# fulcrumgenomics/fgumi

Measured on AMD Instinct MI355X. Metric: simplex consensus throughput, input raw reads/s (depth-8 x 150bp), higher is better.
Workload: dtype f64

## Files before the change

fgumi_amd/csrc/api.cpp:

```cpp
#include <chrono>
#include <cstdio>
#include <stdexcept>
#include <cstring>
#include <mutex>
#include <map>
#include <mutex>
#include <string>
#include <thread>
#include "engine.h"
#include <gnu/libc-version.h>
#include <cmath>
#include "fastpath.h"
#include "host_common.h"
#include "simgen.h"
#include "canon_core.h"
#include "reject_core.h"
#include "aln_tags_core.h"

namespace fgx {
uint32_t launch_canon_molecules(hipStream_t s, bool codec, const canon::Params& P, const canon::CodecParams& PC, const uint8_t* d_blob,
                                const uint64_t* d_rec_off, const uint32_t* d_rec_len, const uint32_t* d_grp_first, const uint32_t* d_def, uint32_t nd,
                                const uint64_t* d_first, uint8_t* d_out, const uint64_t* d_out_off, uint32_t* d_out_len, int* d_status,
                                canon::Delta* d_delta, DevBuf& slabs);
void canon_layout_device(hipStream_t s, const uint32_t* d_rec_len, const uint32_t* d_grp_first, const uint32_t* d_def, uint32_t nd, unsigned long long* work,
// ... 1272 lines not shown
  double run = 0.0;
  for (uint32_t i = 0; i < n; i++) { run += (double)weights[i]; acc[i] = run; }
  const double total = acc[n - 1];
  for (uint32_t k = 1; k < world; k++) {
    const double want = total * (double)k / (double)world;
    const uint32_t idx = (uint32_t)(std::lower_bound(acc.begin(), acc.end(), want) - acc.begin());
    uint32_t c = idx + 1 > n ? n : idx + 1;
    if (c < cuts[k - 1]) c = cuts[k - 1];
    cuts[k] = c;
  }
  cuts[world] = n;
  for (uint32_t k = 1; k <= world; k++) if (cuts[k] < cuts[k - 1]) cuts[k] = cuts[k - 1];
  return 0;
}
uint32_t fgx_debug_last_split_chunks(const fgx_caller* c) { return (c && c->fast) ? c->fast->fp.last_split_chunks : 0u; }
uint32_t fgx_debug_last_big_families(const fgx_caller* c) { return (c && c->fast) ? c->fast->fp.last_big_families : 0u; }
uint32_t fgx_debug_last_meth_device(const fgx_caller* c) { return (c && c->fast) ? c->fast->fp.last_meth_device : 0u; }
uint32_t fgx_debug_last_deep_families(const fgx_caller* c) { return (c && c->fast) ? c->fast->fp.last_deep_families : 0u; }
void fgx_debug_last_split_builds(const fgx_caller* c, uint64_t* out4) {
  if (!out4) return;
  out4[0] = out4[1] = out4[2] = out4[3] = 0;
  if (c && c->fast) { const FastPath& f = c->fast->fp; out4[0] = f.last_packed_families; out4[1] = f.last_classic_families; out4[2] = f.last_split_build; out4[3] = f.last_first_stage_retries; }
}
void fgx_debug_last_chain(const fgx_caller* c, uint32_t* out2) { if (out2) { out2[0] = (c && c->fast) ? c->fast->fp.last_launches : 0u; out2[1] = (c && c->fast) ? c->fast->fp.last_host_syncs : 0u; } }
uint32_t fgx_debug_last_routed(const fgx_caller* c) { return (c && c->fast) ? c->fast->fp.last_routed : 0u; }
int fgx_debug_last_direct(const fgx_caller* c) { return (c && c->fast) ? c->fast->fp.last_direct : 0; }
void fgx_set_general_only(fgx_caller* c, int on) { if (c) c->general_only = on != 0; }
void fgx_set_fast_lds_bytes(fgx_caller* c, uint32_t bytes) { if (c) { if (!c->fast) c->fast = new FastState(); c->fast->fp.lds_tile_bytes_large = bytes; } }

int fgx_call_columns(fgx_caller* c, const uint8_t* bases, const uint8_t* quals, uint32_t n_cols, uint32_t depth, uint8_t* out_base,
                     uint8_t* out_qual, uint32_t* out_depth, uint32_t* out_errors) {
  if (!c) return 1;
  c->err.clear();
  try {
    ColumnBatch& B = c->batch;
    B.clear();
    std::vector<uint8_t> rb, rq;
    for (uint32_t j0 = 0; j0 < n_cols; j0 += 4096) {
      uint32_t w = std::min<uint32_t>(4096, n_cols - j0);
      uint32_t rd0 = (uint32_t)B.reads.size();
      for (uint32_t i = 0; i < depth; i++) {
        rb.resize(w); rq.resize(w);
        for (uint32_t k = 0; k < w; k++) { rb[k] = bases[(size_t)(j0 + k) * depth + i]; rq[k] = quals[(size_t)(j0 + k) * depth + i]; }
        B.add_read(rb.data(), rq.data(), w);
      }
      if (depth == 0) { B.add_job(rd0, 0, w); continue; }
// ... 129 lines not shown
```

fgumi_amd/csrc/fastpath.h:

```cpp
#pragma once
#include "engine.h"

namespace fgx {

constexpr int FAST_RX_CAP = 48;

struct EndDesc {
  uint64_t col_off;
  uint64_t first_off;
  uint64_t kept_off;
  uint32_t cons_len;
  uint32_t rec_size;
  uint16_t mi_off, cb_off;
  uint8_t mi_len, cb_len, rx_len, type;
  uint8_t has_cb, has_rx, valid, meth;
  char rx[FAST_RX_CAP];
};
struct MethSlot { uint32_t std_size, n_ml, mm_len, _pad; };

struct DuplexDesc {
  uint64_t a_off, b_off;
  uint32_t len;
  uint32_t first_rec;
  uint32_t cb_rec;
// ... 158 lines not shown
  uint32_t n_deferred; const uint32_t* d_deferred;
  const uint64_t* d_out_off;
  const uint64_t* d_slot_size;
  uint32_t n_slots;
  double ms_kernels, ms_k_family, ms_k_emit; uint64_t cols_used; uint64_t full_items;
};

struct FastPath {
  DevBuf d_ends, d_sizes, d_offsets, d_code, d_qual, d_depth, d_err, d_misc, d_deferred, d_out, d_scan_tmp, d_strings;
  uint32_t lds_tile_bytes = 12288;
  uint32_t lds_tile_bytes_large = 65536;
  DevBuf d_retry, d_bound, d_colbase, d_statslots, d_full_items, d_full_count, d_obs, d_obs_all, d_retry2, d_retry_old;
  DevBuf d_w2img;
  DevBuf d_famdesc;
  DevBuf d_fwimg;
  DevBuf d_split_rec, d_split_fam, d_split_out, d_route, d_s2img;
  DevBuf d_big;
  uint32_t last_big_families = 0;
  uint32_t last_deep_families = 0;
  DevBuf d_deep_sizes, d_deep_row0, d_deep_rows, d_deep_fams, d_deep_out, d_deep_out2;
  DevBuf d_mflag, d_mu, d_mt, d_mslot, d_mcontigs;
  uint32_t last_meth_device = 0;
  uint32_t last_routed = 0;
  uint64_t last_packed_families = 0, last_classic_families = 0;
  uint32_t last_split_build = 0;
  uint32_t last_first_stage_retries = 0;
  uint32_t last_launches = 0, last_host_syncs = 0;
  DevBuf d_dir_size, d_dir_off, d_dir_base, d_slot_desc, d_slot_err, d_out2, d_scan_tmp2;
  bool direct_off = false;
  uint64_t dir_cap_min = 0;
  uint32_t dir_chunks_run = 0;
  int last_direct = 0;
  uint32_t lds_wave_bytes = 6144;
  uint32_t lds_wave_bytes_duplex = 8704;
  uint32_t lds_wave_bytes_codec = 5120;
  hipEvent_t ev[4] = {nullptr, nullptr, nullptr, nullptr};
  uint32_t pool_slack = 256; bool pool_init = false;
  uint32_t pool_div = 8;
  static constexpr int RUN_AGAIN_LARGER_POOL = -77;
  bool lds_attr_set = false, s2_attr_set = false, v2_attr_set = false;
  static constexpr int MAX_CHUNKS = 65;
  uint32_t last_split_chunks = 0;
  hipStream_t s2 = nullptr;
  hipEvent_t ev_chunk[MAX_CHUNKS] = {}, ev_cols[MAX_CHUNKS] = {}, ev_fin = nullptr, ev_sample = nullptr;
  int run(fgx_caller* c, const uint8_t* d_blob, uint64_t blob_len, const uint64_t* d_rec_off, const uint32_t* d_rec_len, uint32_t n_rec,
          const uint32_t* d_grp_first, uint32_t n_grp, FastResult* res);
// ... 5 lines not shown
```

fgumi_amd/csrc/fastpath.hip:

```cpp
#if !defined(FGX_WAVEMU)
#include <hipcub/hipcub.hpp>
#endif
#include "bamrec.h"
#include "engine.h"
#include <cstdlib>
#include <memory>
#include <string>
#include <type_traits>
#include "fastpath.h"
#include "gate_core.h"
#include "packed_core.h"

#if defined(FGX_WAVEMU)
#define FGX_DYN_LDS(name) uint8_t* const name = wavemu::dyn_lds()
#define FGX_PIN(...) ((void)0)
#define FGX_UNDEF4(a, b, c, d) do { a = 0; b = 0; c = 0; d = 0; } while (0)
#define FGX_MEM_PIN() ((void)0)
#define FGX_CONST_AS
#else
#define FGX_DYN_LDS(name) extern __shared__ __align__(16) uint8_t name[]
#define FGX_PIN(...) asm volatile("" : __VA_ARGS__)
#define FGX_UNDEF4(a, b, c, d) asm volatile("" : "=v"(a), "=v"(b), "=v"(c), "=v"(d))
#define FGX_MEM_PIN() asm volatile("" ::: "memory")
#define FGX_CONST_AS __attribute__((address_space(4)))
#endif

namespace fgx {
// ... 3855 lines not shown
    hip_check(hipcub::DeviceScan::ExclusiveSum(fp.d_scan_tmp.p, tb, in, out, (int)n, s), what);
  }
  template <class Image> const void* table_image(DevBuf& d, void (*build)(Image&, const ConsensusTables&), const char* what) {
    if (!d.p) {
      const auto img = std::make_unique<Image>();
      build(*img, c->h_tables.t);
      d.reserve(sizeof(Image));
      hip_check(hipMemcpyAsync(d.p, img.get(), sizeof(Image), hipMemcpyHostToDevice, s), what);
      sync();
    }
    return d.p;
  }
  FastParams stage_params(uint32_t bytes, bool retry) {
    hip_check(hipMemsetAsync(cnt(MISC_N_RETRY), 0, 4, s), "memset");
    FastParams PS = P;
    PS.group_list = cur_list; PS.lds_wave_bytes = bytes;
    PS.retry = retry ? lists[out_list] : nullptr; PS.n_retry = cnt(MISC_N_RETRY);
    return PS;
  }
  void next_list(uint32_t n) { cur_list = lists[out_list]; n_cur = n; out_list ^= 1; }

  void set_up() {
    fp.last_meth_device = 0; fp.last_direct = 0; fp.last_split_chunks = 0;
    fp.last_routed = 0; fp.last_big_families = 0; fp.last_deep_families = 0; fp.last_packed_families = 0; fp.last_classic_families = 0; fp.last_split_build = 0; fp.last_first_stage_retries = 0;
    fp.d_ends.reserve((size_t)n_slots * (duplex ? sizeof(DuplexDesc) : codec ? sizeof(CodecDesc) : sizeof(EndDesc)));
    fp.d_sizes.reserve(((size_t)n_slots + 1) * 8);
    fp.d_offsets.reserve(((size_t)n_slots + 1) * 8);
    fp.d_deferred.reserve((size_t)n_grp * 4);
    fp.d_misc.reserve(MISC_WORDS * 8);
    hip_check(hipMemsetAsync(fp.d_misc.p, 0, MISC_WORDS * 8, s), "memset");
    misc = fp.d_misc.as<unsigned long long>();
    const std::string strs = c->prefix + c->rg;
    fp.d_strings.reserve(strs.size() + 16);
    if (!strs.empty()) hip_check(hipMemcpyAsync(fp.d_strings.p, strs.data(), strs.size(), hipMemcpyHostToDevice, s), "H2D strings");
    for (int i = 0; i < 4; i++) if (!fp.ev[i]) hip_check(hipEventCreate(&fp.ev[i]), "hipEventCreate");
    fp.d_bound.reserve(((size_t)n_grp + 1) * 8); fp.d_colbase.reserve(((size_t)n_grp + 1) * 8);
    fp.d_statslots.reserve((size_t)STAT_SLOTS * 32 * 8);
    hip_check(hipMemsetAsync(fp.d_statslots.p, 0, (size_t)STAT_SLOTS * 32 * 8, s), "memset");
    fp.d_famdesc.reserve((size_t)n_grp * 16);
    hip_check(hipEventRecord(c->ev0, s), "event");
    hip_check(hipEventRecord(fp.ev[0], s), "event");
    fpw = mean_recs >= 1.0 ? (uint32_t)(64.0 / mean_recs) : 16u;
    fpw = fpw < 1u ? 1u : fpw > 16u ? 16u : fpw;
    if (sw.split_fpw) fpw = sw.split_fpw;
    n_chunks = ps.chunks >= 1 ? (uint32_t)ps.chunks : std::min<uint32_t>(8u, std::max<uint32_t>(1u, n_grp / 150000u));
    if (n_chunks > (uint32_t)FastPath::MAX_CHUNKS - 1) n_chunks = FastPath::MAX_CHUNKS - 1;
    chunk_fam_raw = (n_grp + n_chunks - 1) / n_chunks;
// ... 515 lines not shown
    };
    read_counters();
    if ((duplex || codec) && (uint32_t)h_misc[MISC_N_SLOW] != 0) {
      if (codec) FGX_LAUNCH(k_emit_codec, wave_per_slot, dim3(256), 0, s, CE);
      else if (meth_dup) FGX_LAUNCH(HIP_KERNEL_NAME(k_emit_duplex<1>), wave_per_slot, dim3(256), 0, s, DE);
      else if (dup_cap) FGX_LAUNCH(HIP_KERNEL_NAME(k_emit_duplex<0, 1>), wave_per_slot, dim3(256), 0, s, DE);
      else FGX_LAUNCH(HIP_KERNEL_NAME(k_emit_duplex<0>), wave_per_slot, dim3(256), 0, s, DE);
      read_counters();
    }
    float ms = 0, msf = 0, mse = 0;
    hip_check(hipEventElapsedTime(&ms, c->ev0, c->ev1), "elapsed");
    hip_check(hipEventElapsedTime(&msf, fp.ev[0], fp.ev[1]), "elapsed");
    hip_check(hipEventElapsedTime(&mse, fp.ev[2], fp.ev[3]), "elapsed");
    res->d_out = out_ptr;
    res->out_len = out_len;
    res->count = h_misc[MISC_STATS + 1];
    for (int i = 0; i < FGX_STATS_LEN; i++) res->stats[i] = h_misc[MISC_STATS + i];
    res->n_deferred = (uint32_t)(h_misc[MISC_N_DEFERRED] & 0xFFFFFFFFull);
    res->d_deferred = fp.d_deferred.as<uint32_t>();
    res->d_out_off = fp.d_offsets.as<uint64_t>();
    res->d_slot_size = fp.d_sizes.as<uint64_t>();
    res->n_slots = n_slots;
    res->ms_kernels = ms; res->ms_k_family = msf; res->ms_k_emit = mse;
    fp.last_packed_families = h_misc[MISC_BUILD_FAMILIES]; fp.last_classic_families = h_misc[MISC_BUILD_FAMILIES + 1];
    res->cols_used = h_misc[MISC_COLS_USED];
    res->full_items = n_full;
  }
};

int run_once(FastPath& fp, fgx_caller* c, const uint8_t* d_blob, uint64_t blob_len, const uint64_t* d_rec_off, const uint32_t* d_rec_len, uint32_t n_rec,
             const uint32_t* d_grp_first, uint32_t n_grp, FastResult* res) {
  memset(res, 0, sizeof(*res));
  fp.last_launches = 0; fp.last_host_syncs = 0;
  if (n_grp == 0) return 0;
  static const ProcessSwitches ps{};
  Batch b{fp, c, d_blob, blob_len, d_rec_off, d_rec_len, n_rec, d_grp_first, n_grp, res, ps};
  b.set_up();
  b.parse_first_chunk_early();
  b.bound_columns();
  b.fill_params();
  if (b.use_split) b.split_pipeline();
  if (b.simplex_v2) b.wave2_chain();
  b.family_wave_stages();
  b.deep_families();
  b.workgroup_families();
  if (const int rc = b.call_full()) return rc;
  if (b.direct) if (const int rc = b.check_direct()) return rc;
// ... 41 lines not shown
```

fgumi_amd/csrc/packed_core.h:

```cpp
#pragma once
#include <cstdint>
#include "consensus_math.h"

namespace fgx {
namespace pk {

constexpr uint32_t H = 0x80808080u;

FGX_HD uint32_t perm(uint32_t a, uint32_t b, uint32_t sel) {
#if defined(__HIP_DEVICE_COMPILE__)
  return __builtin_amdgcn_perm(a, b, sel);
#else
  const unsigned long long src = ((unsigned long long)a << 32) | b;
  uint32_t r = 0;
  for (int i = 0; i < 4; i++) {
    const uint32_t s = (sel >> (8 * i)) & 0xFFu;
    const uint32_t byte = s < 8u ? (uint32_t)(src >> (8 * s)) & 0xFFu : 0u;
    r |= byte << (8 * i);
  }
  return r;
#endif
}
FGX_HD uint32_t bitrev32(uint32_t x) {
#if defined(__HIP_DEVICE_COMPILE__)
// ... 9 lines not shown
  const uint32_t nv = lenE > 8u * k ? lenE - 8u * k : 0u;
  if (nv < 8u) { const unsigned long long f = ~(0x8080808080808080ull << (8u * nv)); *nfl &= (uint32_t)f; *nfh &= (uint32_t)(f >> 32); }
}
FGX_HD bool any_below(uint32_t qx, uint32_t qy, uint32_t mb4, uint32_t nfl, uint32_t nfh) {
  return ((((qx - mb4) & ~qx & nfl) | ((qy - mb4) & ~qy & nfh))) != 0u;
}
FGX_HD uint32_t keep_mask(uint32_t qx, uint32_t qy, uint32_t mb4) {
  const uint32_t gl = ((qx | H) - mb4) | qx, gh = ((qy | H) - mb4) | qy;
  uint32_t keep = 0;
  keep |= (uint32_t)((int32_t)(gl << 24) >> 31) & 0x000000F0u; keep |= (uint32_t)((int32_t)(gl << 16) >> 31) & 0x0000000Fu;
  keep |= (uint32_t)((int32_t)(gl << 8) >> 31) & 0x0000F000u;  keep |= (uint32_t)((int32_t)gl >> 31) & 0x00000F00u;
  keep |= (uint32_t)((int32_t)(gh << 24) >> 31) & 0x00F00000u; keep |= (uint32_t)((int32_t)(gh << 16) >> 31) & 0x000F0000u;
  keep |= (uint32_t)((int32_t)(gh << 8) >> 31) & 0xF0000000u;  keep |= (uint32_t)((int32_t)gh >> 31) & 0x0F000000u;
  return keep;
}

struct Acc { uint32_t f_or, A8, B8; };
FGX_HD void acc_reset(Acc& a) { a.f_or = 0; a.A8 = 0; a.B8 = 0; }
FGX_HD void acc_row(Acc& a, uint32_t qx, uint32_t qy, uint32_t b, uint32_t mb4, uint32_t nfl, uint32_t nfh) {
  if (any_below(qx, qy, mb4, nfl, nfh)) b &= keep_mask(qx, qy, mb4);
  a.f_or |= b;
  const uint32_t nz = (((b & 0x77777777u) + 0x77777777u) | b) & 0x88888888u;
  a.A8 += nz & 0x08080808u; a.B8 += (nz >> 4) & 0x08080808u;
}

struct Out { uint32_t code2[2], qual2[2], dep4[4], flag2[2], valid2[2]; int32_t c_lo, lo_s, hi_s; };
FGX_HD void finalize(const Acc& a, bool inl, bool lrev, uint32_t lenE, uint32_t cntE, uint32_t k, uint32_t nsafe, uint32_t cap, uint32_t min_cons_bq, uint32_t min_reads, Out& o) {
  uint32_t f_or = a.f_or, Ce = a.A8 >> 3, Co = a.B8 >> 3;
  if (lrev) { f_or = bitrev32(f_or); const uint32_t t = __builtin_bswap32(Ce); Ce = __builtin_bswap32(Co); Co = t; }
  o.c_lo = lrev ? (int32_t)lenE - 8 - 8 * (int32_t)k : 8 * (int32_t)k;
  const int32_t hi_r = (int32_t)cntE - o.c_lo;
  o.lo_s = o.c_lo < 0 ? -o.c_lo : 0; o.hi_s = !inl || hi_r < 0 ? 0 : hi_r > 8 ? 8 : hi_r;
  unsigned long long V = 0;
  if (o.hi_s > o.lo_s) {
    const unsigned long long hiM = o.hi_s >= 8 ? ~0ull : (1ull << (8 * o.hi_s)) - 1ull, loM = (1ull << (8 * (o.lo_s > 7 ? 7 : o.lo_s))) - 1ull;
    V = hiM & ~loM & 0x8080808080808080ull;
  }
  const uint32_t N4 = nsafe * 0x01010101u;
  const bool cap_lt = cap < min_cons_bq;
  const uint32_t QA4 = (cap_lt ? (uint32_t)FGX_MIN_PHRED : cap) * 0x01010101u, QZ4 = (min_reads > 0u ? 0u : (uint32_t)FGX_MIN_PHRED) * 0x01010101u;
#pragma unroll
  for (int h = 0; h < 2; h++) {
    const uint32_t Pb = perm(f_or, f_or, h ? 0x03030202u : 0x01010000u);
    const uint32_t O = ((Pb >> 4) & 0x000F000Fu) | (Pb & 0x0F000F00u);
    const uint32_t C = perm(Ce, Co, h ? 0x07030602u : 0x05010400u);
    const uint32_t Vh = h ? (uint32_t)(V >> 32) : (uint32_t)V;
// ... 50 lines not shown
```

fgumi_amd/csrc/simplex_split.inc:

```

#ifndef FGX_S2_OCC
#define FGX_S2_OCC 6
#endif
#ifndef FGX_S2_OCC_PACKED
#define FGX_S2_OCC_PACKED 7
#endif
#ifndef FGX_S2_PAIRS
#define FGX_S2_PAIRS 256
#endif

#ifndef FGX_S2_F32
#define FGX_S2_F32 1
#endif
#ifndef FGX_S2_FMASEL
#define FGX_S2_FMASEL 1
#endif
#ifndef FGX_S2_NOSUM
#define FGX_S2_NOSUM 1
#endif
#ifndef FGX_S2_PREGATE
#define FGX_S2_PREGATE 1
#endif
struct S2Lds {
  GateTables g;
  uint8_t t1[96];
  alignas(16) float pairf[FGX_S2_PAIRS][2];
  alignas(16) double pair[FGX_S2_PAIRS][2];
};
// ... 525 lines not shown
#endif
#define S2_PIN4(a_, b_, c_, d_) FGX_PIN("+v"(a_.x), "+v"(a_.y), "+v"(b_.x), "+v"(b_.y), "+v"(c_.x), "+v"(c_.y), "+v"(d_.x), "+v"(d_.y))
#define S2_PIN1(a_) FGX_PIN("+v"(a_.x), "+v"(a_.y))
#define S2_OBSERVE_FAST(q_, sb_) do { \
    const uint32_t w_c = __builtin_amdgcn_ubfe((uint32_t)(sb_), ish, 4u); \
    const bool w_g = (uint32_t)(q_) >= min_bq; \
    const uint32_t w_t = w_g ? w_c : 0u; \
    f_or |= w_t; f_sum += w_t; f_cnt += w_g ? 1u : 0u; \
  } while (0)

typedef unsigned short s2_u16x2 __attribute__((ext_vector_type(2)));
__device__ __forceinline__ uint32_t s2_pkmax(uint32_t a, uint32_t b) { s2_u16x2 x, y; __builtin_memcpy(&x, &a, 4); __builtin_memcpy(&y, &b, 4); x = __builtin_elementwise_max(x, y); uint32_t r; __builtin_memcpy(&r, &x, 4); return r; }
__device__ __forceinline__ uint32_t s2_pkmin(uint32_t a, uint32_t b) { s2_u16x2 x, y; __builtin_memcpy(&x, &a, 4); __builtin_memcpy(&y, &b, 4); x = __builtin_elementwise_min(x, y); uint32_t r; __builtin_memcpy(&r, &x, 4); return r; }
__device__ __forceinline__ void s2_st16(uint8_t* p, uint32_t v) { const uint16_t w = (uint16_t)v; __builtin_memcpy(p, &w, 2); }
struct S2DirRec { uint32_t base, Lc, type, fk, kept, o_seq, o_qual, o_rg, o_t3, o_cd, o_ce, o_mi, o_cb, o_rx, size, hcb, cbl; };

__device__ uint32_t g_s2_dbg[64];
constexpr uint32_t S2_PACKED_MAX_ROWS = 31;
__device__ __forceinline__ bool s2_packed_shape(uint32_t m_a, uint32_t m_b, uint32_t len_a, uint32_t len_b, uint32_t nsafe) {
  const bool oa = m_a < 2u || (m_a >= nsafe && m_a <= S2_PACKED_MAX_ROWS), ob = m_b < 2u || (m_b >= nsafe && m_b <= S2_PACKED_MAX_ROWS);
  return oa && ob && ((len_a + 7u) >> 3) + ((len_b + 7u) >> 3) <= 64u;
}

constexpr uint32_t S2_PAD_FRONT = 8;
__host__ __device__ __forceinline__ uint32_t s2_padded_b(uint32_t lc_a) { return S2_PAD_FRONT + ((lc_a + 7u) & ~7u) + 16u; }
static_assert(COL_BOUND_PAD >= S2_PAD_FRONT + 7 + 16 + 7 + 8, "the column bound's padding covers the packed build's layout: 8 + r8(lc_a) + 16 + r8(lc_b) + 8 <= 2 lc + 2 + COL_BOUND_PAD");
template <int COLS> struct S2SharedOf {
#if FGX_S2_F32
  typedef typename std::conditional<COLS == 1, S2Tiny, S2Head>::type type;
#else
  typedef S2Lds type;
#endif
};
typedef uint32_t s2_u32x4 __attribute__((ext_vector_type(4)));
template <int QS_T, int SS_T, int DIRECT, int COLS, bool FUSED>
__device__ __forceinline__ void s2_cols_family(const FastParams& P, const uint32_t g, bool bail, const uint32_t tiny_w, const s2_u32x4* const im, uint8_t* const W,
                                               typename S2SharedOf<COLS>::type& sL, const uint32_t lane, const uint32_t my_list) {
  typedef typename S2SharedOf<COLS>::type S2Shared;
  typedef s2_u32x4 u32x4;
  auto& sT = sL.g;
  constexpr bool TINY = FGX_S2_F32 && COLS == 1;
  constexpr uint32_t IMG_V = TINY ? 0u : (uint32_t)((FGX_S2_F32 ? S2_HEAD_BYTES : (uint32_t)sizeof(S2Lds)) / 16);
  const unsigned long long below = (1ull << lane) - 1ull;
  (void)sT; (void)IMG_V; (void)tiny_w; (void)im; (void)below;

  const uint4 fd = P.fam_desc[g];
// ... 47 lines not shown
  const bool act = !bail && lane < n;
  u32x4 d0 = {0, 0, 0, 0}, d1 = {0, 0, 0, 0};
  if (act) { const u32x4* rp = (const u32x4*)&P.split_rec[r0 + lane]; d0 = rp[0]; d1 = rp[1]; }
  if constexpr (!FUSED) {
    if constexpr (TINY) {
      if (threadIdx.x < 24u) ((uint32_t*)&sL.t1[0])[threadIdx.x] = tiny_w;
      else if (threadIdx.x == 24u) sL.g.cap = tiny_w;
    } else {
      u32x4* const img_dst = (u32x4*)&sL;
#pragma unroll
      for (int u = 0; u < 6; u++) { const uint32_t ii = threadIdx.x + u * blockDim.x; if (ii < IMG_V) img_dst[ii] = im[u]; }
    }
  }
  const uint32_t body_off = d0.x, seq_rel = d0.y & 0xFFFF, l_seq = d0.y >> 16, clip = d0.z & 0xFFFF, ov_off1 = d0.z >> 16;
  const uint32_t ov_off2 = d0.w & 0xFFFF, ov_cnt = d0.w >> 16;
  const uint32_t slot = d1.x & 0xFF, mate_slot = (d1.x >> 8) & 0xFF, bits = (d1.x >> 16) & 0xFF, cb_len = d1.x >> 24;
  const uint32_t cb_rel = d1.y & 0xFFFF, mi_rel = d1.y >> 16, mi_len = d1.z & 0xFF, rx_rel = d1.z >> 16;
  const uint32_t ty = bits & 3u;
  const bool rev = (bits & 4u) != 0, has_cb = (bits & 8u) != 0;
  const unsigned long long lo_off = uniform_u64((unsigned long long)fd.x | ((unsigned long long)fd.y << 32));
  const uint8_t* const fbase = P.blob + lo_off;
  const uint32_t S0 = n * QS;
  if (act) *(uint2*)(W + ibase + 8u * slot) = make_uint2(body_off + seq_rel, l_seq);
  if constexpr (FUSED) wave_sync(); else __syncthreads();
  if (bail) return;
  {
    const uint32_t cpr = qc + sc, total = n * cpr;
    for (uint32_t t0 = 0; t0 < total; t0 += 256) {
      u32x4 v[4];
      uint32_t dst[4];
      bool on[4];
#pragma unroll
      for (int u = 0; u < 4; u++) {
        const uint32_t t = t0 + 64u * u + lane;
        const bool in = t < total;
        const uint32_t tt = in ? t : 0u;
        const uint32_t row = s2_mul24(tt, inv_cpr) >> 24;
        const uint32_t ch = tt - s2_mul24(row, cpr);
        const uint2 e = *(const uint2*)(W + ibase + 8u * row);
        const bool isq = ch < qc;
        const uint32_t c = isq ? ch : ch - qc;
        const uint32_t sbytes = (e.y + 1u) >> 1;
        const uint32_t src = e.x + (isq ? sbytes : 0u) + 16u * c;
        dst[u] = (isq ? row * QS : S0 + row * SS) + 16u * c;
        on[u] = in;
        const bool need_ld = in && 16u * c < (isq ? e.y : sbytes);
        u32x4 x = {0, 0, 0, 0};
        if (need_ld) __builtin_memcpy(&x, fbase + src, 16);
        v[u] = x;
      }
#pragma unroll
      for (int u = 0; u < 4; u++) if (on[u]) *(u32x4*)(W + dst[u]) = v[u];
    }
  }
  wave_sync();
  PH(1)
  const uint32_t my_q = slot * QS, my_s = S0 + slot * SS;
  if (__any(act && W[my_q] == 0xFF)) { to_route(); return; }
  S2_ABLATE_AFTER(1, W[my_s])

  const uint32_t min_bq = uni((uint32_t)P.min_input_bq & 0xFFu);
  uint32_t ov_agree = 0, ov_dis = 0, ov_corr = 0;
  {
    auto shared_base = [&](const bool in, const uint32_t o1, const uint32_t o2, const uint32_t q1, const uint32_t q2, const uint32_t sh1, const uint32_t sh2) {
      const uint32_t c1 = ((uint32_t)W[o1] >> sh1) & 15, c2 = ((uint32_t)W[o2] >> sh2) & 15;
      const uint32_t qa = W[q1], qb = W[q2];
      const bool valid = in && (c1 > c2 ? c1 : c2) != 15;
      const bool agree = c1 == c2;
      const uint32_t sm = qa + qb, nq = sm < 93 ? sm : 93;
      const int32_t d = (int32_t)qa - (int32_t)qb;
      const uint32_t ad = (uint32_t)(d < 0 ? -d : d), dq = ad < FGX_MIN_PHRED ? (uint32_t)FGX_MIN_PHRED : ad;
      const uint32_t cb = d == 0 ? 15u : d > 0 ? c1 : c2;
      const uint32_t newq = agree ? nq : dq;
      const bool drop = newq < min_bq;
      const uint32_t x1 = drop ? c1 : agree ? 0u : (c1 ^ cb), x2 = drop ? c2 : agree ? 0u : (c2 ^ cb);
// ... 397 lines not shown
  auto run_cols_packed = [&](const uint32_t cnt_a, const uint32_t cnt_b, const uint32_t m, const bool last_run) -> bool {
    const uint32_t nsafe = P.s2_nsafe;
    const uint32_t ga = cnt_a ? (len_a + 7u) >> 3 : 0u, gb = cnt_b ? (len_b + 7u) >> 3 : 0u;
    const bool dbg = (P.s2_packed & 2u) != 0;
    if (!(P.s2_packed && m >= nsafe && m <= S2_PACKED_MAX_ROWS && P.min_reads <= nsafe && min_bq <= 128u && ((QS & 7u) | (SS & 3u)) == 0u && ga + gb <= 64u &&
          S0 + s2_mul24(n, SS) < 65536u && lc_a + lc_b < 65536u)) {
      if (dbg && lane == 0) atomicAdd(&g_s2_dbg[42], 1u);
      return false;
    }
    if (dbg && lane == 0) atomicAdd(&g_s2_dbg[0], 1u);
    const bool in_b = lane >= ga, inl = lane < ga + gb;
    const uint32_t k = inl ? (in_b ? lane - ga : lane) : 0u;
    const bool lrev = (in_b ? rev_b : rev_a) != 0;
    const uint32_t lenE = in_b ? len_b : len_a, cntE = in_b ? cnt_b : cnt_a;
    const uint32_t rowE = in_b ? m_a : 0u;
    const uint32_t qaddr0 = s2_mul24(rowE, QS) + 8u * k, saddr0 = S0 + s2_mul24(rowE, SS) + 4u * k;
    const uint32_t H = pk::H;
    uint32_t nfl, nfh;
    pk::count_masks(lenE, k, &nfl, &nfh);
    const uint32_t mb4 = min_bq * 0x01010101u;
    pk::Acc A;
    pk::acc_reset(A);
    {
      uint32_t qj = qaddr0, sj = saddr0, j = 0;
      for (; j + 4 <= m; j += 4, qj += 4 * QS, sj += 4 * SS) {
        const uint2 q0 = *(const uint2*)(W + qj), q1 = *(const uint2*)(W + qj + QS), q2 = *(const uint2*)(W + qj + 2 * QS), q3 = *(const uint2*)(W + qj + 3 * QS);
        const uint32_t b0 = *(const uint32_t*)(W + sj), b1_ = *(const uint32_t*)(W + sj + SS), b2_ = *(const uint32_t*)(W + sj + 2 * SS), b3_ = *(const uint32_t*)(W + sj + 3 * SS);
        pk::acc_row(A, q0.x, q0.y, b0, mb4, nfl, nfh); pk::acc_row(A, q1.x, q1.y, b1_, mb4, nfl, nfh);
        pk::acc_row(A, q2.x, q2.y, b2_, mb4, nfl, nfh); pk::acc_row(A, q3.x, q3.y, b3_, mb4, nfl, nfh);
      }
      for (; j < m; j++, qj += QS, sj += SS) { const uint2 q0 = *(const uint2*)(W + qj); const uint32_t b0 = *(const uint32_t*)(W + sj); pk::acc_row(A, q0.x, q0.y, b0, mb4, nfl, nfh); }
    }
    PH(9)
    pk::Out F;
    pk::finalize(A, inl, lrev, lenE, cntE, k, nsafe, sT.cap, P.min_cons_bq, P.min_reads, F);
    const int32_t c_lo = F.c_lo, lo_s = F.lo_s, hi_s = F.hi_s;
    const uint32_t* const code2 = F.code2; const uint32_t* const qual2 = F.qual2; const uint32_t* const dep4 = F.dep4;
    const uint32_t* const flag2 = F.flag2; const uint32_t* const full2 = F.valid2;
    PH(10)
    uint32_t fm = (flag2[0] >> 7) | (flag2[1] >> 3);
    const uint32_t fc = (uint32_t)__builtin_popcount(fm);
    const unsigned long long pb0 = __ballot((fc & 1u) != 0), pb1 = __ballot((fc & 2u) != 0), pb2 = __ballot((fc & 4u) != 0), pb3 = __ballot((fc & 8u) != 0);
    const uint32_t T = uni((uint32_t)__popcll(pb0) + 2u * (uint32_t)__popcll(pb1) + 4u * (uint32_t)__popcll(pb2) + 8u * (uint32_t)__popcll(pb3));
    const uint32_t oc0 = (in_b ? offB : offA) + (uint32_t)c_lo;
    const uint32_t list = (P.lds_wave_bytes - 8u * T) & ~7u;
    if (T && (8u * T + 8u > P.lds_wave_bytes || ibase + s2_mul24(icnt, (uint32_t)sizeof(FullItem)) > list)) {
      if (dbg && lane == 0) atomicAdd(&g_s2_dbg[3], 1u);
      gone = true; return true;
    }
    (void)last_run;
    (void)full2; (void)lo_s;
    if (hi_s > lo_s) {
      const uint2 cv = make_uint2(code2[0], code2[1]), qv = make_uint2(qual2[0], qual2[1]);
      const u32x4 dv = {dep4[0], dep4[1], dep4[2], dep4[3]}, zv = {0u, 0u, 0u, 0u};
// ... 192 lines not shown
  constexpr uint32_t IMG_V = TINY ? 0u : (uint32_t)((FGX_S2_F32 ? S2_HEAD_BYTES : (uint32_t)sizeof(S2Lds)) / 16);
  static_assert(IMG_V <= 6 * 64 || !FGX_S2_F32, "table image larger than six loads per thread");
  const u32x4* const img_src = (const u32x4*)P.s2_image;
  u32x4 im[6];
  uint32_t tiny_w = 0;
  if constexpr (TINY) {
    static_assert(offsetof(S2Lds, t1) % 4 == 0 && offsetof(GateTables, cap) % 4 == 0, "the packed build copies its tables as 32-bit words");
    const uint32_t* const w = (const uint32_t*)P.s2_image;
    if (threadIdx.x < 24u) tiny_w = w[offsetof(S2Lds, t1) / 4 + threadIdx.x];
    else if (threadIdx.x == 24u) tiny_w = w[(offsetof(S2Lds, g) + offsetof(GateTables, cap)) / 4];
  } else {
#pragma unroll
    for (int u = 0; u < 6; u++) { const uint32_t ii = threadIdx.x + u * blockDim.x; im[u] = img_src[ii < IMG_V ? ii : 0u]; }
  }
  uint8_t* W = dyn + (size_t)wv * P.lds_wave_bytes;
  const uint32_t my_list = blockIdx.x & (N_LISTS - 1);
  s2_cols_family<QS_T, SS_T, DIRECT, COLS, false>(P, g, bail, tiny_w, im, W, sL, lane, my_list);
}

__global__ __launch_bounds__(256) void k_split_finish(FastParams P, uint32_t count) {
  typedef uint32_t u32x4 __attribute__((ext_vector_type(4)));
  const uint32_t gi = blockIdx.x * blockDim.x + threadIdx.x;
  const uint32_t lane = threadIdx.x & 63;
  uint32_t c_total = 0, c_cons = 0, c_insuf = 0, c_zero = 0, c_orphan = 0, c_agree = 0, c_dis = 0, c_corr = 0, c_packed = 0, c_classic = 0;
  if (gi < count) {
    const uint32_t g = P.group_list ? P.group_list[gi] : P.g0 + gi;
    const SplitOut O = P.split_out[g];
    const uint32_t slot0 = 3 * g;
    const uint32_t o_status = O.status & 0x7Fu;
    const bool padded = (O.status & 0x80u) != 0;
    if (o_status == 2) { c_total = O.n; c_insuf = O.n; }
    const bool direct = P.out != nullptr;
    if (o_status != 0 && !direct) {
      EndDesc* D = &P.ends[slot0];
      D[0].valid = 0; D[1].valid = 0; D[2].valid = 0;
      P.rec_sizes[slot0] = 0; P.rec_sizes[slot0 + 1] = 0; P.rec_sizes[slot0 + 2] = 0;
    }
    if (o_status == 1) {
      c_packed = padded ? 1u : 0u; c_classic = padded ? 0u : 1u;
      c_total = O.n; c_cons = O.ne;
      c_insuf = O.rej & 0xFF; c_zero = (O.rej >> 8) & 0xFF; c_orphan = O.rej >> 16;
      c_agree = O.ov_agree; c_dis = O.ov_dis; c_corr = O.ov_corr;
      const uint4 fd = P.fam_desc[g];
      const unsigned long long lo_off = (unsigned long long)fd.x | ((unsigned long long)fd.y << 32);
      const uint32_t r0 = P.grp_first[g];
      const SplitFam F = P.split_fam[g];
      const SplitRec R0 = P.split_rec[r0];
      const uint64_t col_base = P.col_base[g];
      if (direct) {
        const uint8_t* const fbase = P.blob + lo_off;
        const uint8_t* const strs = (const uint8_t*)P.strings;
        const uint32_t mi0 = R0.mi_len, nm = P.prefix_len + 1u + mi0;
        const uint8_t* const mi_src = fbase + R0.mi_rel;
        uint64_t rec_off = P.dir_off[g];
        for (uint32_t k = 0; k < O.ne; k++) {
          const uint32_t Lc = k == 0 ? O.lc_a : O.lc_b, e_type = k == 0 ? O.type_a : 2u;
          const uint32_t fk = k == 0 ? O.fk_a : O.fk_b, kept = k == 0 ? O.kept_a : O.kept_b;
          const uint32_t dst = k == 0 ? O.depth_stats & 0xFFFFu : O.depth_stats >> 16, maxd = dst & 0xFFu, mind = dst >> 8;
          const SplitRec RK = P.split_rec[r0 + fk];
          const bool hcb = P.cell0 && (RK.bits & 8u);
          const uint32_t cbl = RK.cb_len, rxn = F.rx_all ? kept : 0u, rxl = F.rx_len;
          const uint32_t o_seq = 36u + nm + 1u, o_rg = o_seq + ((Lc + 1u) >> 1) + Lc, o_t3 = o_rg + 3u + P.rg_len + 1u;
          const uint32_t o_cd = o_t3 + 15u + 8u, o_ce = o_cd + 2u * Lc + 8u, o_mi = P.per_base_tags ? o_ce + 2u * Lc : o_t3 + 15u;
          const uint32_t o_cb = o_mi + 3u + mi0 + 1u, o_rx = o_cb + (hcb ? 3u + cbl + 1u : 0u), size = o_rx + (rxn ? 3u + rxl + 1u : 0u);
// ... 65 lines not shown
            for (uint32_t bb = 0; bb < 4; bb++) {
              const uint32_t ch = (v >> (8 * bb)) & 0xFF, up = ch & 0xDFu, idx = up - 'A';
              const bool dna = idx < 26 && ((0x00082045u >> idx) & 1u);
              const uint32_t o = (4 * w + bb < rx_ulen) ? ((rx_cnt > 1 && dna) ? up : ch) : 0u;
              out |= o << (8 * bb);
            }
          }
          rxw[w] = out;
        }
        const uint64_t col_off = col_base + (padded ? (k == 0 ? S2_PAD_FRONT : s2_padded_b(O.lc_a)) : (k == 0 ? 0u : (uint32_t)O.lc_a)), kept_off = lo_off + RK.body_off;
        const u32x4 p0 = {(uint32_t)col_off, (uint32_t)(col_off >> 32), (uint32_t)lo_off, (uint32_t)(lo_off >> 32)};
        const u32x4 p1 = {(uint32_t)kept_off, (uint32_t)(kept_off >> 32), Lc, size};
        const u32x4 p2 = {(uint32_t)R0.mi_rel | ((uint32_t)RK.cb_rel << 16), mi0_len | (cbl << 8) | (rx_ulen << 16) | (e_type << 24),
                          (hcb ? 1u : 0u) | ((rx_cnt ? 1u : 0u) << 8) | (1u << 16), rxw[0]};
        const u32x4 p3 = {rxw[1], rxw[2], rxw[3], rxw[4]}, p4 = {rxw[5], rxw[6], rxw[7], rxw[8]}, p5 = {rxw[9], rxw[10], rxw[11], 0u};
        u32x4* dst = (u32x4*)&P.ends[slot0 + e_type];
        dst[0] = p0; dst[1] = p1; dst[2] = p2; dst[3] = p3; dst[4] = p4; dst[5] = p5;
        P.rec_sizes[slot0 + e_type] = (uint64_t)size + 4;
      }
    }
  }
  const uint32_t t_cons = wave_sum(c_cons), t_total = wave_sum(c_total), t_insuf = wave_sum(c_insuf), t_zero = wave_sum(c_zero), t_orphan = wave_sum(c_orphan);
  const uint32_t t_agree = wave_sum(c_agree), t_dis = wave_sum(c_dis), t_corr = wave_sum(c_corr);
  const uint32_t t_packed = wave_sum(c_packed), t_classic = wave_sum(c_classic);
  if (lane == 0) {
    unsigned long long* st = P.stats + (size_t)((blockIdx.x * 4 + (threadIdx.x >> 6)) & (STAT_SLOTS - 1)) * 32;
    if (t_total) atomicAdd(&st[0], (unsigned long long)t_total);
    if (t_cons) atomicAdd(&st[1], (unsigned long long)t_cons);
    const uint32_t filt = t_insuf + t_zero + t_orphan;
    if (filt) atomicAdd(&st[2], (unsigned long long)filt);
    if (t_insuf) atomicAdd(&st[3 + FGX_REJ_INSUFFICIENT_READS], (unsigned long long)t_insuf);
    if (t_zero) atomicAdd(&st[3 + FGX_REJ_ZERO_LENGTH_AFTER_TRIMMING], (unsigned long long)t_zero);
    if (t_orphan) atomicAdd(&st[3 + FGX_REJ_ORPHAN_CONSENSUS], (unsigned long long)t_orphan);
    if (t_agree + t_dis) atomicAdd(&st[24], (unsigned long long)(t_agree + t_dis));
    if (t_agree) atomicAdd(&st[25], (unsigned long long)t_agree);
    if (t_dis) atomicAdd(&st[26], (unsigned long long)t_dis);
    if (t_corr) atomicAdd(&st[27], (unsigned long long)t_corr);
    if (t_packed) atomicAdd(&st[28], (unsigned long long)t_packed);
    if (t_classic) atomicAdd(&st[29], (unsigned long long)t_classic);
  }
}
```

Baseline: 2.902 billion.

## Flag low-quality rows during packed load and skip quality reads for clean rows

While staging packed family rows into LDS, each row's quality bytes are checked against the minimum input base quality and a per-family bitmask of rows with any sub-floor base is recorded with an atomic OR. The accumulation loop then uses a cheaper clean-row accumulate that skips the quality load and masking for rows without low-quality bases, and falls back to the full path only for flagged rows. The packed occupancy define is lowered from 7 to 6, presumably to make room for the extra registers. This adds per-chunk flag computation and LDS atomics during loading, and emits a new floor-row statistic.

Result: no change. 2.884 billion (median of 3 runs) (-0.6%).

```diff
diff --git a/fgumi_amd/csrc/api.cpp b/fgumi_amd/csrc/api.cpp
--- a/fgumi_amd/csrc/api.cpp
+++ b/fgumi_amd/csrc/api.cpp
@@ -1318,6 +1318,7 @@
   out4[0] = out4[1] = out4[2] = out4[3] = 0;
   if (c && c->fast) { const FastPath& f = c->fast->fp; out4[0] = f.last_packed_families; out4[1] = f.last_classic_families; out4[2] = f.last_split_build; out4[3] = f.last_first_stage_retries; }
 }
+uint64_t fgx_debug_last_packed_floor_rows(const fgx_caller* c) { return (c && c->fast) ? c->fast->fp.last_packed_floor_rows : 0ull; }
 void fgx_debug_last_chain(const fgx_caller* c, uint32_t* out2) { if (out2) { out2[0] = (c && c->fast) ? c->fast->fp.last_launches : 0u; out2[1] = (c && c->fast) ? c->fast->fp.last_host_syncs : 0u; } }
 uint32_t fgx_debug_last_routed(const fgx_caller* c) { return (c && c->fast) ? c->fast->fp.last_routed : 0u; }
 int fgx_debug_last_direct(const fgx_caller* c) { return (c && c->fast) ? c->fast->fp.last_direct : 0; }
diff --git a/fgumi_amd/csrc/fastpath.h b/fgumi_amd/csrc/fastpath.h
--- a/fgumi_amd/csrc/fastpath.h
+++ b/fgumi_amd/csrc/fastpath.h
@@ -204,6 +204,7 @@
   DevBuf d_mflag, d_mu, d_mt, d_mslot, d_mcontigs;
   uint32_t last_meth_device = 0;
   uint32_t last_routed = 0;
+  uint64_t last_packed_floor_rows = 0;
   uint64_t last_packed_families = 0, last_classic_families = 0;
   uint32_t last_split_build = 0;
   uint32_t last_first_stage_retries = 0;
diff --git a/fgumi_amd/csrc/fastpath.hip b/fgumi_amd/csrc/fastpath.hip
--- a/fgumi_amd/csrc/fastpath.hip
+++ b/fgumi_amd/csrc/fastpath.hip
@@ -3,6 +3,9 @@
 #endif
 #include "bamrec.h"
 #include "engine.h"
+#if defined(FGX_WAVEMU)
+#include <cassert>
+#endif
 #include <cstdlib>
 #include <memory>
 #include <string>
@@ -3904,7 +3907,7 @@
 
   void set_up() {
     fp.last_meth_device = 0; fp.last_direct = 0; fp.last_split_chunks = 0;
-    fp.last_routed = 0; fp.last_big_families = 0; fp.last_deep_families = 0; fp.last_packed_families = 0; fp.last_classic_families = 0; fp.last_split_build = 0; fp.last_first_stage_retries = 0;
+    fp.last_routed = 0; fp.last_big_families = 0; fp.last_deep_families = 0; fp.last_packed_families = 0; fp.last_classic_families = 0; fp.last_packed_floor_rows = 0; fp.last_split_build = 0; fp.last_first_stage_retries = 0;
     fp.d_ends.reserve((size_t)n_slots * (duplex ? sizeof(DuplexDesc) : codec ? sizeof(CodecDesc) : sizeof(EndDesc)));
     fp.d_sizes.reserve(((size_t)n_slots + 1) * 8);
     fp.d_offsets.reserve(((size_t)n_slots + 1) * 8);
@@ -4466,7 +4469,7 @@
     res->d_slot_size = fp.d_sizes.as<uint64_t>();
     res->n_slots = n_slots;
     res->ms_kernels = ms; res->ms_k_family = msf; res->ms_k_emit = mse;
-    fp.last_packed_families = h_misc[MISC_BUILD_FAMILIES]; fp.last_classic_families = h_misc[MISC_BUILD_FAMILIES + 1];
+    fp.last_packed_families = h_misc[MISC_BUILD_FAMILIES]; fp.last_classic_families = h_misc[MISC_BUILD_FAMILIES + 1]; fp.last_packed_floor_rows = h_misc[MISC_BUILD_FAMILIES + 2];
     res->cols_used = h_misc[MISC_COLS_USED];
     res->full_items = n_full;
   }
diff --git a/fgumi_amd/csrc/packed_core.h b/fgumi_amd/csrc/packed_core.h
--- a/fgumi_amd/csrc/packed_core.h
+++ b/fgumi_amd/csrc/packed_core.h
@@ -55,6 +55,25 @@
   a.f_or |= b;
   const uint32_t nz = (((b & 0x77777777u) + 0x77777777u) | b) & 0x88888888u;
   a.A8 += nz & 0x08080808u; a.B8 += (nz >> 4) & 0x08080808u;
+}
+
+FGX_HD void acc_row_clean(Acc& a, uint32_t b) {
+  a.f_or |= b;
+  const uint32_t nz = (((b & 0x77777777u) + 0x77777777u) | b) & 0x88888888u;
+  a.A8 += nz & 0x08080808u; a.B8 += (nz >> 4) & 0x08080808u;
+}
+FGX_HD uint32_t floor_flags(uint32_t x0, uint32_t x1, uint32_t x2, uint32_t x3, uint32_t mb4) {
+  return (((x0 - mb4) & ~x0) | ((x1 - mb4) & ~x1) | ((x2 - mb4) & ~x2) | ((x3 - mb4) & ~x3)) & H;
+}
+FGX_HD bool floor_hit(uint32_t x0, uint32_t x1, uint32_t x2, uint32_t x3, uint32_t mb4, uint32_t nv) {
+  const uint32_t x[4] = {x0, x1, x2, x3};
+  uint32_t f = 0;
+  for (uint32_t w = 0; w < 4; w++) {
+    const uint32_t v = nv > 4u * w ? nv - 4u * w : 0u;
+    const uint32_t keep = v >= 4u ? H : H & ((1u << (8u * v)) - 1u);
+    f |= (x[w] - mb4) & ~x[w] & keep;
+  }
+  return f != 0u;
 }
 
 struct Out { uint32_t code2[2], qual2[2], dep4[4], flag2[2], valid2[2]; int32_t c_lo, lo_s, hi_s; };
diff --git a/fgumi_amd/csrc/simplex_split.inc b/fgumi_amd/csrc/simplex_split.inc
--- a/fgumi_amd/csrc/simplex_split.inc
+++ b/fgumi_amd/csrc/simplex_split.inc
@@ -3,7 +3,7 @@
 #define FGX_S2_OCC 6
 #endif
 #ifndef FGX_S2_OCC_PACKED
-#define FGX_S2_OCC_PACKED 7
+#define FGX_S2_OCC_PACKED 6
 #endif
 #ifndef FGX_S2_PAIRS
 #define FGX_S2_PAIRS 256
@@ -575,6 +575,18 @@
   return oa && ob && ((len_a + 7u) >> 3) + ((len_b + 7u) >> 3) <= 64u;
 }
 
+#if defined(FGX_WAVEMU)
+static inline bool s2_same_counted(const pk::Acc& x, const pk::Acc& y, uint32_t nfl, uint32_t nfh) {
+  uint32_t nm = 0, am = 0, bm = 0;
+  for (uint32_t p = 0; p < 8; p++) {
+    if (!(((p < 4 ? nfl >> (8 * p + 7) : nfh >> (8 * (p - 4) + 7))) & 1u)) continue;
+    const uint32_t nib = p ^ 1u;
+    nm |= 0xFu << (4 * nib);
+    if (nib & 1u) bm |= 0xFFu << (8 * (nib >> 1)); else am |= 0xFFu << (8 * (nib >> 1));
+  }
+  return ((x.f_or ^ y.f_or) & nm) == 0u && ((x.A8 ^ y.A8) & am) == 0u && ((x.B8 ^ y.B8) & bm) == 0u;
+}
+#endif
 constexpr uint32_t S2_PAD_FRONT = 8;
 __host__ __device__ __forceinline__ uint32_t s2_padded_b(uint32_t lc_a) { return S2_PAD_FRONT + ((lc_a + 7u) & ~7u) + 16u; }
 static_assert(COL_BOUND_PAD >= S2_PAD_FRONT + 7 + 16 + 7 + 8, "the column bound's padding covers the packed build's layout: 8 + r8(lc_a) + 16 + r8(lc_b) + 8 <= 2 lc + 2 + COL_BOUND_PAD");
@@ -668,10 +680,13 @@
   const uint8_t* const fbase = P.blob + lo_off;
   const uint32_t S0 = n * QS;
   if (act) *(uint2*)(W + ibase + 8u * slot) = make_uint2(body_off + seq_rel, l_seq);
+  const uint32_t low_rows_at = need + 8u;
+  if constexpr (COLS == 1) { if (!bail && lane == 0) *(unsigned long long*)(W + low_rows_at) = 0ull; }
   if constexpr (FUSED) wave_sync(); else __syncthreads();
   if (bail) return;
   {
     const uint32_t cpr = qc + sc, total = n * cpr;
+    const uint32_t mb4 = ((uint32_t)P.min_input_bq & 0xFFu) * 0x01010101u;
     for (uint32_t t0 = 0; t0 < total; t0 += 256) {
       u32x4 v[4];
       uint32_t dst[4];
@@ -697,6 +712,23 @@
       }
 #pragma unroll
       for (int u = 0; u < 4; u++) if (on[u]) *(u32x4*)(W + dst[u]) = v[u];
+      if constexpr (COLS == 1) {
+        uint32_t fl[4];
+#pragma unroll
+        for (int u = 0; u < 4; u++) fl[u] = (on[u] && dst[u] < S0) ? pk::floor_flags(v[u].x, v[u].y, v[u].z, v[u].w, mb4) : 0u;
+        if ((fl[0] | fl[1]) | (fl[2] | fl[3])) {
+#pragma unroll
+          for (int u = 0; u < 4; u++) {
+            if (fl[u]) {
+              const uint32_t t = t0 + 64u * u + lane;
+              const uint32_t row = s2_mul24(t, inv_cpr) >> 24, ch = t - s2_mul24(row, cpr);
+              const uint32_t ls = *(const uint32_t*)(W + ibase + 8u * row + 4u);
+              const uint32_t nv = ls > 16u * ch ? ls - 16u * ch : 0u;
+              if (pk::floor_hit(v[u].x, v[u].y, v[u].z, v[u].w, mb4, nv)) atomicOr((unsigned long long*)(W + low_rows_at), 1ull << row);
+            }
+          }
+        }
+      }
     }
   }
   wave_sync();
@@ -1140,14 +1172,40 @@
     pk::Acc A;
     pk::acc_reset(A);
     {
+      const unsigned long long low_rows = uniform_u64(*(const unsigned long long*)(W + low_rows_at));
+      const uint32_t lowm = uni(((cnt_a ? (uint32_t)low_rows : 0u) | (cnt_b ? (uint32_t)(low_rows >> m_a) : 0u)) & ((1u << m) - 1u));
+      rej += (uint32_t)__builtin_popcount(lowm) << 24;
+      auto row = [&](const uint32_t jr, const uint32_t qa, const uint32_t sa) {
+        const uint32_t b = *(const uint32_t*)(W + sa);
+        if ((lowm >> jr) & 1u) { const uint2 q = *(const uint2*)(W + qa); pk::acc_row(A, q.x, q.y, b, mb4, nfl, nfh); }
+        else {
+#if defined(FGX_WAVEMU)
+          pk::Acc A2 = A;
+          const uint2 q = *(const uint2*)(W + qa);
+          pk::acc_row(A2, q.x, q.y, b, mb4, nfl, nfh);
+#endif
+          pk::acc_row_clean(A, b);
+#if defined(FGX_WAVEMU)
+          if (inl) assert(s2_same_counted(A2, A, nfl, nfh));
+#endif
+        }
+      };
       uint32_t qj = qaddr0, sj = saddr0, j = 0;
       for (; j + 4 <= m; j += 4, qj += 4 * QS, sj += 4 * SS) {
-        const uint2 q0 = *(const uint2*)(W + qj), q1 = *(const uint2*)(W + qj + QS), q2 = *(const uint2*)(W + qj + 2 * QS), q3 = *(const uint2*)(W + qj + 3 * QS);
-        const uint32_t b0 = *(const uint32_t*)(W + sj), b1_ = *(const uint32_t*)(W + sj + SS), b2_ = *(const uint32_t*)(W + sj + 2 * SS), b3_ = *(const uint32_t*)(W + sj + 3 * SS);
-        pk::acc_row(A, q0.x, q0.y, b0, mb4, nfl, nfh); pk::acc_row(A, q1.x, q1.y, b1_, mb4, nfl, nfh);
-        pk::acc_row(A, q2.x, q2.y, b2_, mb4, nfl, nfh); pk::acc_row(A, q3.x, q3.y, b3_, mb4, nfl, nfh);
-      }
-      for (; j < m; j++, qj += QS, sj += SS) { const uint2 q0 = *(const uint2*)(W + qj); const uint32_t b0 = *(const uint32_t*)(W + sj); pk::acc_row(A, q0.x, q0.y, b0, mb4, nfl, nfh); }
+        if (((lowm >> j) & 15u) == 0u) {
+#if defined(FGX_WAVEMU)
+          row(j, qj, sj); row(j + 1, qj + QS, sj + SS); row(j + 2, qj + 2 * QS, sj + 2 * SS); row(j + 3, qj + 3 * QS, sj + 3 * SS);
+#else
+          const uint32_t b0 = *(const uint32_t*)(W + sj), b1_ = *(const uint32_t*)(W + sj + SS), b2_ = *(const uint32_t*)(W + sj + 2 * SS), b3_ = *(const uint32_t*)(W + sj + 3 * SS);
+          pk::acc_row_clean(A, b0); pk::acc_row_clean(A, b1_); pk::acc_row_clean(A, b2_); pk::acc_row_clean(A, b3_);
+#endif
+        } else {
+#pragma unroll 1
+          for (uint32_t i = 0; i < 4; i++) row(j + i, qj + i * QS, sj + i * SS);
+        }
+      }
+#pragma unroll 1
+      for (; j < m; j++, qj += QS, sj += SS) row(j, qj, sj);
     }
     PH(9)
     pk::Out F;
@@ -1386,7 +1444,7 @@
   typedef uint32_t u32x4 __attribute__((ext_vector_type(4)));
   const uint32_t gi = blockIdx.x * blockDim.x + threadIdx.x;
   const uint32_t lane = threadIdx.x & 63;
-  uint32_t c_total = 0, c_cons = 0, c_insuf = 0, c_zero = 0, c_orphan = 0, c_agree = 0, c_dis = 0, c_corr = 0, c_packed = 0, c_classic = 0;
+  uint32_t c_total = 0, c_cons = 0, c_insuf = 0, c_zero = 0, c_orphan = 0, c_agree = 0, c_dis = 0, c_corr = 0, c_packed = 0, c_classic = 0, c_floor = 0;
   if (gi < count) {
     const uint32_t g = P.group_list ? P.group_list[gi] : P.g0 + gi;
     const SplitOut O = P.split_out[g];
@@ -1403,7 +1461,7 @@
     if (o_status == 1) {
       c_packed = padded ? 1u : 0u; c_classic = padded ? 0u : 1u;
       c_total = O.n; c_cons = O.ne;
-      c_insuf = O.rej & 0xFF; c_zero = (O.rej >> 8) & 0xFF; c_orphan = O.rej >> 16;
+      c_insuf = O.rej & 0xFF; c_zero = (O.rej >> 8) & 0xFF; c_orphan = (O.rej >> 16) & 0xFF; c_floor = O.rej >> 24;
       c_agree = O.ov_agree; c_dis = O.ov_dis; c_corr = O.ov_corr;
       const uint4 fd = P.fam_desc[g];
       const unsigned long long lo_off = (unsigned long long)fd.x | ((unsigned long long)fd.y << 32);
@@ -1515,6 +1573,7 @@
   }
   const uint32_t t_cons = wave_sum(c_cons), t_total = wave_sum(c_total), t_insuf = wave_sum(c_insuf), t_zero = wave_sum(c_zero), t_orphan = wave_sum(c_orphan);
   const uint32_t t_agree = wave_sum(c_agree), t_dis = wave_sum(c_dis), t_corr = wave_sum(c_corr);
+  const uint32_t t_floor = wave_sum(c_floor);
   const uint32_t t_packed = wave_sum(c_packed), t_classic = wave_sum(c_classic);
   if (lane == 0) {
     unsigned long long* st = P.stats + (size_t)((blockIdx.x * 4 + (threadIdx.x >> 6)) & (STAT_SLOTS - 1)) * 32;
@@ -1531,5 +1590,6 @@
     if (t_corr) atomicAdd(&st[27], (unsigned long long)t_corr);
     if (t_packed) atomicAdd(&st[28], (unsigned long long)t_packed);
     if (t_classic) atomicAdd(&st[29], (unsigned long long)t_classic);
+    if (t_floor) atomicAdd(&st[30], (unsigned long long)t_floor);
   }
 }
```
